# BurnhamG/PyTorch-ScalableFHVAE

Hardware: AMD Instinct MI355X
Metric: segments/sec + ELBO (nats/frame), (B,20,80) fbank (higher is better)
Workload: dtype bf16; 1 GPU; c3: fhvae.FHVAE 2x256 LSTM enc/dec, z1=z2=32, 28k-seq mu2 table, batch 2048; per-GPU batch 2048, T=20, F=80, full train step (fwd+loss+bwd+Adam), intended objective, mu_idx uniform; global_batch=2048, parallelism=single

## Files before the change

pytorch-scalablefhvae_amd/csrc/lstm_bwd_rs.hip:

```cpp
#include <cstdlib>

#include "lstm_cluster_dev.h"
#include "trace.h"

namespace fh {

namespace {

constexpr int kH = 256, kG = 4 * kH, kHU = 64, kNU = 4;
constexpr int kKS = 8;

template <int RT>
__device__ __forceinline__ int rs_xoff(int par, int cluster, int src, int j, int wave, int rt) {
  return ((((((par * 64 + cluster) * kNU + src) * 3 + (j - 1)) * 4 + wave) * RT + rt) << 9);
}

template <int RT>
struct RsCfg {
  static constexpr int SMEM = RT * 16 * 512;
};

template <int RT, bool UM>
__global__ __launch_bounds__(kThreads) void lstm_bwd_layer_rs_kernel(ClBwd p) {
  constexpr int H = kH, G = kG;
  extern __shared__ __attribute__((aligned(16))) char smem[];
  char* Img = smem;
  const int tid = threadIdx.x, lane = tid & 63, wave = tid >> 6;
  const int r = lane & 15, q = lane >> 4;

  const int joined = cluster_join(p.sync, (int*)Img);
  if (joined < 0) return;
  const int info = joined & 255;
  const unsigned ep0 = (unsigned)(joined >> 8) * kSeqEpochs;
  const int cluster = (info >> 5) * (32 / kNU) + (info & 31) / kNU, me = (info & 31) % kNU;
  const int r0 = p.row0 + cluster * p.Mc;
  const int rend = min(p.row0 + p.nrows, r0 + p.Mc);
  if (r0 >= rend) return;
  unsigned* flags = p.sync + kSyncFlags + cluster * 32;
  const int u0 = me * kHU;
  const int uq = u0 + wave * 16 + q * 4;
  const int B = p.B, T = p.T;

  int row[RT];
  int64_t rowc[RT];
#pragma unroll
  for (int rt = 0; rt < RT; ++rt) {
    row[rt] = r0 + rt * 16 + r;
    rowc[rt] = row[rt] < rend ? row[rt] : rend - 1;
  }
  f32x4 dcreg[RT], ccur[RT], dgs[RT][4], own[RT];
#pragma unroll
  for (int rt = 0; rt < RT; ++rt) {
    dcreg[rt] = ccur[rt] = own[rt] = f32x4{0.f, 0.f, 0.f, 0.f};
#pragma unroll
    for (int g = 0; g < 4; ++g) dgs[rt][g] = f32x4{0.f, 0.f, 0.f, 0.f};
  }
  const __amdgpu_buffer_rsrc_t x_rs = make_rsrc(p.xch);
  const float* ext_src = p.d_hs_top;
  int ibase[4], wbase[2];
#pragma unroll
  for (int k3 = 0; k3 < 4; ++k3) {
    ibase[k3] = r * 512 + (((k3 * 4 + q) ^ r) << 4);
  }
#pragma unroll
  for (int g1 = 0; g1 < 2; ++g1)
    wbase[g1] = r * 512 + (((g1 * 8 + 2 * wave + (q >> 1)) ^ r) << 4) + (q & 1) * 8;
  unsigned long long* tl = (p.tlog && cluster == 0 && me == 0) ? p.tlog + (p.tlog_slot ? 256 : 0) : nullptr;
  CL_TLOG(6);

  uint2 gkn[RT][4];
  f32x4 cprevn[RT], extn[RT], ccurn[RT];
  typedef unsigned u32x4v __attribute__((ext_vector_type(4)));
  const bool nt = p.nt != 0;
  auto ld16 = [&](const void* q) -> uint4 {
    if (nt) {
      const u32x4v v = __builtin_nontemporal_load((const u32x4v*)q);
      return uint4{v.x, v.y, v.z, v.w};
    }
    return *(const uint4*)q;
  };
  auto ldf4 = [&](const float* q) -> f32x4 { return nt ? __builtin_nontemporal_load((const f32x4*)q) : *(const f32x4*)q; };
  auto load_epi = [&](int sn) {
    const int t = T - 1 - sn;
#pragma unroll
    for (int rt = 0; rt < RT; ++rt) {
      if constexpr (UM) {
        const u16* gp = p.gates + ((int64_t)t * B + rowc[rt]) * G + uq * 4;
        const uint4 a = ld16(gp), b = ld16(gp + 8);
        gkn[rt][0] = uint2{a.x, a.y}, gkn[rt][1] = uint2{a.z, a.w}, gkn[rt][2] = uint2{b.x, b.y}, gkn[rt][3] = uint2{b.z, b.w};
      } else {
        cl_load_gates(p.gates + ((int64_t)t * B + rowc[rt]) * G, uq, gkn[rt]);
      }
      if (sn == 0) ccurn[rt] = *(const f32x4*)(p.cs + ((int64_t)t * B + rowc[rt]) * H + uq);
      cprevn[rt] = t > 0 ? ldf4(p.cs + ((int64_t)(t - 1) * B + rowc[rt]) * H + uq) : f32x4{0.f, 0.f, 0.f, 0.f};
      f32x4 e = f32x4{0.f, 0.f, 0.f, 0.f};
      if (ext_src) e = ldf4(ext_src + ((int64_t)t * B + rowc[rt]) * H + uq);
      if (sn == 0 && p.d_hn) e += *(const f32x4*)(p.d_hn + rowc[rt] * p.hn_ld + uq);
      extn[rt] = e;
    }
  };
  __syncthreads();
  bf16x8 wreg[kKS][kNU];
#pragma unroll
  for (int ks = 0; ks < kKS; ++ks)
#pragma unroll
    for (int j = 0; j < kNU; ++j) {
      const int unit = ((me + j) & 3) * kHU + wave * 16 + r;
      const int col = (ks >> 1) * H + u0 + (ks & 1) * 32 + q * 8;
      wreg[ks][j] = __builtin_bit_cast(bf16x8, *(const uint4*)(p.w_hh_t[0] + (int64_t)unit * G + col));
    }
  load_epi(0);
  CL_TLOG(7);
  for (int s = 0; s < T; ++s) {
    CL_TLOG(s * 8 + 0);
    const int t = T - 1 - s;
    f32x4 dh[RT];
    CL_TLOG(s * 8 + 1);
    uint2 pin[RT][3];
    if (s > 0) {
      if (!cluster_wait(p.sync, flags, kNU, ep0 + (unsigned)s)) return;
      CL_TLOG(s * 8 + 2);
#pragma unroll
      for (int jj = 1; jj < kNU; ++jj)
#pragma unroll
        for (int rt = 0; rt < RT; ++rt) {
          const u32x2 v = __builtin_amdgcn_raw_buffer_load_b64(x_rs, rs_xoff<RT>((s - 1) & 1, cluster, (me - jj) & 3, jj, wave, rt) + lane * 8, 0, kSc1);
          pin[rt][jj - 1] = uint2{v.x, v.y};
        }
    }
    uint2 gk[RT][4];
    f32x4 cprev[RT];
#pragma unroll
    for (int rt = 0; rt < RT; ++rt) {
#pragma unroll
      for (int g = 0; g < 4; ++g) gk[rt][g] = gkn[rt][g];
      cprev[rt] = cprevn[rt];
      dh[rt] = extn[rt] + own[rt];
      if (s == 0) ccur[rt] = ccurn[rt];
    }
    if (s > 0) {
#pragma unroll
      for (int rt = 0; rt < RT; ++rt)
#pragma unroll
        for (int j = 0; j < 3; ++j) dh[rt] += unpack4(pin[rt][j]);
    }
    __builtin_amdgcn_sched_barrier(0);
    if (s + 1 < T) load_epi(s + 1);
    uint2 dpk[RT][4];
#pragma unroll
    for (int rt = 0; rt < RT; ++rt) {
      f32x4 ig, fg, gg, og;
      if constexpr (UM) {
#pragma unroll
        for (int i = 0; i < 4; ++i) {
          ig[i] = bf2f((u16)(gk[rt][i].x & 0xffff)), fg[i] = bf2f((u16)(gk[rt][i].x >> 16));
          gg[i] = bf2f((u16)(gk[rt][i].y & 0xffff)), og[i] = bf2f((u16)(gk[rt][i].y >> 16));
        }
      } else {
        ig = unpack4(gk[rt][0]), fg = unpack4(gk[rt][1]), gg = unpack4(gk[rt][2]), og = unpack4(gk[rt][3]);
      }
      f32x4 dp[4];
#pragma unroll
      for (int i = 0; i < 4; ++i) {
        const float tc = tanhf_(ccur[rt][i]);
        float dc = dh[rt][i] * og[i] * (1.f - tc * tc);
        if (s > 0) dc += dcreg[rt][i];
        const float d_o = dh[rt][i] * tc;
        const float d_i = dc * gg[i], d_f = dc * cprev[rt][i], d_g = dc * ig[i];
        dcreg[rt][i] = dc * fg[i];
        dp[0][i] = d_i * ig[i] * (1.f - ig[i]);
        dp[1][i] = d_f * fg[i] * (1.f - fg[i]);
        dp[2][i] = d_g * (1.f - gg[i] * gg[i]);
        dp[3][i] = d_o * og[i] * (1.f - og[i]);
      }
      ccur[rt] = cprev[rt];
      const bool live = row[rt] < rend;
#pragma unroll
      for (int g = 0; g < 4; ++g) {
        if (live) dgs[rt][g] += dp[g];
        dpk[rt][g] = pack4(dp[g]);
        *(uint2*)(Img + wbase[g & 1] + (g >> 1) * 256 + rt * 8192) = dpk[rt][g];
      }
    }
    asm volatile("s_waitcnt lgkmcnt(0)\n\ts_barrier" ::: "memory");
    CL_TLOG(s * 8 + 3);
    if (s + 1 < T) {
      f32x4 acc[RT][kNU];
#pragma unroll
      for (int rt = 0; rt < RT; ++rt)
#pragma unroll
        for (int j = 0; j < kNU; ++j) acc[rt][j] = f32x4{0.f, 0.f, 0.f, 0.f};
      bf16x8 bfrag[2][RT];
      auto ifrag = [&](int ks, int buf) {
#pragma unroll
        for (int rt = 0; rt < RT; ++rt)
          bfrag[buf][rt] = __builtin_bit_cast(bf16x8, *(const uint4*)(Img + ibase[ks & 3] + (ks >> 2) * 256 + rt * 8192));
      };
      ifrag(0, 0);
      __builtin_amdgcn_sched_group_barrier(0x100, RT, 0);
#pragma unroll
      for (int ks = 0; ks < kKS; ++ks) {
        if (ks + 1 < kKS) ifrag(ks + 1, (ks + 1) & 1);
#pragma unroll
        for (int j = 0; j < kNU; ++j)
#pragma unroll
          for (int rt = 0; rt < RT; ++rt) acc[rt][j] = __builtin_amdgcn_mfma_f32_16x16x32_bf16(wreg[ks][j], bfrag[ks & 1][rt], acc[rt][j], 0, 0, 0);
        if (ks + 1 < kKS) {
          __builtin_amdgcn_sched_group_barrier(0x008, 1, 0);
          __builtin_amdgcn_sched_group_barrier(0x100, RT, 0);
          __builtin_amdgcn_sched_group_barrier(0x008, RT * kNU - 1, 0);
        } else {
          __builtin_amdgcn_sched_group_barrier(0x008, RT * kNU, 0);
        }
      }
#pragma unroll
      for (int rt = 0; rt < RT; ++rt) {
        own[rt] = acc[rt][0];
#pragma unroll
        for (int j = 1; j < kNU; ++j)
          *(uint2*)((char*)p.xch + rs_xoff<RT>(s & 1, cluster, me, j, wave, rt) + lane * 8) = pack4(acc[rt][j]);
      }
    }
    auto img_chunk = [&](int i) -> uint4 {
      const int c = (wave * RT * 2 + i) * 64 + lane;
      return *(const uint4*)(Img + kc_off<32>(c >> 5, c & 31));
    };
    const uint4 v0 = img_chunk(0), v1 = img_chunk(1), v2 = RT > 1 ? img_chunk(2) : uint4{0u, 0u, 0u, 0u},
                v3 = RT > 1 ? img_chunk(3) : uint4{0u, 0u, 0u, 0u};
    CL_TLOG(s * 8 + 4);
    if (s + 1 < T) cluster_publish(flags, me, ep0 + (unsigned)(s + 1));
    else __syncthreads();
    CL_TLOG(s * 8 + 5);
    auto dg_store = [&](int i, const uint4& v) {
      const int c = (wave * RT * 2 + i) * 64 + lane;
      const int rw = r0 + (c >> 5), cc = c & 31;
      if (rw < rend) {
        u16* dst = p.dg + ((int64_t)t * B + rw) * G + (cc >> 3) * H + u0 + (cc & 7) * 8;
        if (nt)
          __builtin_nontemporal_store(u32x4v{v.x, v.y, v.z, v.w}, (u32x4v*)dst);
        else
          *(uint4*)dst = v;
      }
    };
    dg_store(0, v0);
    dg_store(1, v1);
    if constexpr (RT > 1) {
      dg_store(2, v2);
      dg_store(3, v3);
    }
  }
  if (p.d_xc_zero && me == 0 && wave == 0) {
#pragma unroll
    for (int rt = 0; rt < RT; ++rt)
      if (row[rt] < rend)
        for (int c = q; c < p.Ic; c += 4) p.d_xc_zero[(int64_t)row[rt] * p.Ic + c] = 0.f;
  }
#pragma unroll
  for (int g = 0; g < 4; ++g) {
    f32x4 vs = f32x4{0.f, 0.f, 0.f, 0.f};
#pragma unroll
    for (int rt = 0; rt < RT; ++rt) {
      vs += dgs[rt][g];
      if (p.dgsum && row[rt] < rend) *(f32x4*)(p.dgsum + (int64_t)row[rt] * G + g * H + uq) = dgs[rt][g];
    }
    if (p.db_ih[0] || p.db_hh[0]) db_reduce_add(vs, p.db_ih[0], p.db_hh[0], g * H + uq, lane);
  }
  CL_TLOG((T - 1) * 8 + 7);
}

template <int RT>
int launch_rs(const ClBwd& p, hipStream_t st) {
  if (p.gates_um)
    hipLaunchKernelGGL((lstm_bwd_layer_rs_kernel<RT, true>), dim3(kGrid), dim3(kThreads), RsCfg<RT>::SMEM, st, p);
  else
    hipLaunchKernelGGL((lstm_bwd_layer_rs_kernel<RT, false>), dim3(kGrid), dim3(kThreads), RsCfg<RT>::SMEM, st, p);
  return fh_launch_status();
}

}

int cluster_bwd_layer_rs(const ClBwd& p, hipStream_t st) {
  if (p.NU != kNU || p.Mc > 32 || p.Mc % 16 != 0) return FHVAE_ERR_SHAPE;
  return p.Mc <= 16 ? launch_rs<1>(p, st) : launch_rs<2>(p, st);
}

}
```

Baseline: 1.264 million segments/s.

## Restructure LSTM backward step to precompute gate factors off the critical path

Reorganizes the LSTM backward recurrence so the gate-dependent factors (tanh, sigmoid derivatives, cprev products) are computed for the next step right after its loads are issued, leaving only a few FMAs that depend on the incoming dh. The first timestep is peeled via a compile-time flag, the accumulator zeroing is folded into the first MFMA, and the live-row masking moves out of the loop to the final reduction. The c and ext loads now go through buffer resource descriptors with a zero-range trick for t=0 and a null ext, and the non-temporal load/store path is hardcoded in place of the runtime flag. This raises register pressure from the precomputed factor arrays and removes the option of normal cached accesses.

After: 1.253 million segments/s (median of 2 runs). No clear change (-0.9%).

```diff
diff --git a/pytorch-scalablefhvae_amd/csrc/lstm_bwd_rs.hip b/pytorch-scalablefhvae_amd/csrc/lstm_bwd_rs.hip
--- a/pytorch-scalablefhvae_amd/csrc/lstm_bwd_rs.hip
+++ b/pytorch-scalablefhvae_amd/csrc/lstm_bwd_rs.hip
@@ -1,4 +1,5 @@
 #include <cstdlib>
+#include <type_traits>
 
 #include "lstm_cluster_dev.h"
 #include "trace.h"
@@ -48,10 +49,10 @@
     row[rt] = r0 + rt * 16 + r;
     rowc[rt] = row[rt] < rend ? row[rt] : rend - 1;
   }
-  f32x4 dcreg[RT], ccur[RT], dgs[RT][4], own[RT];
+  f32x4 dcreg[RT], dgs[RT][4], own[RT];
 #pragma unroll
   for (int rt = 0; rt < RT; ++rt) {
-    dcreg[rt] = ccur[rt] = own[rt] = f32x4{0.f, 0.f, 0.f, 0.f};
+    dcreg[rt] = own[rt] = f32x4{0.f, 0.f, 0.f, 0.f};
 #pragma unroll
     for (int g = 0; g < 4; ++g) dgs[rt][g] = f32x4{0.f, 0.f, 0.f, 0.f};
   }
@@ -69,19 +70,21 @@
   CL_TLOG(6);
 
   uint2 gkn[RT][4];
-  f32x4 cprevn[RT], extn[RT], ccurn[RT];
+  f32x4 cprevn[RT], extn[RT], ccur[RT];
   typedef unsigned u32x4v __attribute__((ext_vector_type(4)));
-  const bool nt = p.nt != 0;
   auto ld16 = [&](const void* q) -> uint4 {
-    if (nt) {
-      const u32x4v v = __builtin_nontemporal_load((const u32x4v*)q);
-      return uint4{v.x, v.y, v.z, v.w};
-    }
-    return *(const uint4*)q;
+    const u32x4v v = __builtin_nontemporal_load((const u32x4v*)q);
+    return uint4{v.x, v.y, v.z, v.w};
   };
-  auto ldf4 = [&](const float* q) -> f32x4 { return nt ? __builtin_nontemporal_load((const f32x4*)q) : *(const f32x4*)q; };
+  int coff[RT];
+#pragma unroll
+  for (int rt = 0; rt < RT; ++rt) coff[rt] = (int)((rowc[rt] * H + uq) * 4);
   auto load_epi = [&](int sn) {
     const int t = T - 1 - sn;
+    const __amdgpu_buffer_rsrc_t cs_rs = __builtin_amdgcn_make_buffer_rsrc(const_cast<float*>(p.cs + (int64_t)(t > 0 ? t - 1 : 0) * B * H), 0,
+                                                                            t > 0 ? B * H * 4 : 0, 0x00020000);
+    const __amdgpu_buffer_rsrc_t ext_rs = __builtin_amdgcn_make_buffer_rsrc(const_cast<float*>(ext_src ? ext_src + (int64_t)t * B * H : p.cs), 0,
+                                                                             ext_src ? B * H * 4 : 0, 0x00020000);
 #pragma unroll
     for (int rt = 0; rt < RT; ++rt) {
       if constexpr (UM) {
@@ -91,62 +94,12 @@
       } else {
         cl_load_gates(p.gates + ((int64_t)t * B + rowc[rt]) * G, uq, gkn[rt]);
       }
-      if (sn == 0) ccurn[rt] = *(const f32x4*)(p.cs + ((int64_t)t * B + rowc[rt]) * H + uq);
-      cprevn[rt] = t > 0 ? ldf4(p.cs + ((int64_t)(t - 1) * B + rowc[rt]) * H + uq) : f32x4{0.f, 0.f, 0.f, 0.f};
-      f32x4 e = f32x4{0.f, 0.f, 0.f, 0.f};
-      if (ext_src) e = ldf4(ext_src + ((int64_t)t * B + rowc[rt]) * H + uq);
-      if (sn == 0 && p.d_hn) e += *(const f32x4*)(p.d_hn + rowc[rt] * p.hn_ld + uq);
-      extn[rt] = e;
+      cprevn[rt] = __builtin_bit_cast(f32x4, __builtin_amdgcn_raw_buffer_load_b128(cs_rs, coff[rt], 0, 2));
+      extn[rt] = __builtin_bit_cast(f32x4, __builtin_amdgcn_raw_buffer_load_b128(ext_rs, coff[rt], 0, 2));
     }
   };
-  __syncthreads();
-  bf16x8 wreg[kKS][kNU];
-#pragma unroll
-  for (int ks = 0; ks < kKS; ++ks)
-#pragma unroll
-    for (int j = 0; j < kNU; ++j) {
-      const int unit = ((me + j) & 3) * kHU + wave * 16 + r;
-      const int col = (ks >> 1) * H + u0 + (ks & 1) * 32 + q * 8;
-      wreg[ks][j] = __builtin_bit_cast(bf16x8, *(const uint4*)(p.w_hh_t[0] + (int64_t)unit * G + col));
-    }
-  load_epi(0);
-  CL_TLOG(7);
-  for (int s = 0; s < T; ++s) {
-    CL_TLOG(s * 8 + 0);
-    const int t = T - 1 - s;
-    f32x4 dh[RT];
-    CL_TLOG(s * 8 + 1);
-    uint2 pin[RT][3];
-    if (s > 0) {
-      if (!cluster_wait(p.sync, flags, kNU, ep0 + (unsigned)s)) return;
-      CL_TLOG(s * 8 + 2);
-#pragma unroll
-      for (int jj = 1; jj < kNU; ++jj)
-#pragma unroll
-        for (int rt = 0; rt < RT; ++rt) {
-          const u32x2 v = __builtin_amdgcn_raw_buffer_load_b64(x_rs, rs_xoff<RT>((s - 1) & 1, cluster, (me - jj) & 3, jj, wave, rt) + lane * 8, 0, kSc1);
-          pin[rt][jj - 1] = uint2{v.x, v.y};
-        }
-    }
-    uint2 gk[RT][4];
-    f32x4 cprev[RT];
-#pragma unroll
-    for (int rt = 0; rt < RT; ++rt) {
-#pragma unroll
-      for (int g = 0; g < 4; ++g) gk[rt][g] = gkn[rt][g];
-      cprev[rt] = cprevn[rt];
-      dh[rt] = extn[rt] + own[rt];
-      if (s == 0) ccur[rt] = ccurn[rt];
-    }
-    if (s > 0) {
-#pragma unroll
-      for (int rt = 0; rt < RT; ++rt)
-#pragma unroll
-        for (int j = 0; j < 3; ++j) dh[rt] += unpack4(pin[rt][j]);
-    }
-    __builtin_amdgcn_sched_barrier(0);
-    if (s + 1 < T) load_epi(s + 1);
-    uint2 dpk[RT][4];
+  f32x4 pA[RT], pPo[RT], pPi[RT], pPf[RT], pPg[RT], pF[RT], base[RT];
+  auto prep = [&](const uint2 (&gk)[RT][4], const f32x4 (&cprev)[RT], const f32x4 (&ext)[RT]) {
 #pragma unroll
     for (int rt = 0; rt < RT; ++rt) {
       f32x4 ig, fg, gg, og;
@@ -159,37 +112,95 @@
       } else {
         ig = unpack4(gk[rt][0]), fg = unpack4(gk[rt][1]), gg = unpack4(gk[rt][2]), og = unpack4(gk[rt][3]);
       }
-      f32x4 dp[4];
 #pragma unroll
       for (int i = 0; i < 4; ++i) {
         const float tc = tanhf_(ccur[rt][i]);
-        float dc = dh[rt][i] * og[i] * (1.f - tc * tc);
-        if (s > 0) dc += dcreg[rt][i];
-        const float d_o = dh[rt][i] * tc;
-        const float d_i = dc * gg[i], d_f = dc * cprev[rt][i], d_g = dc * ig[i];
-        dcreg[rt][i] = dc * fg[i];
-        dp[0][i] = d_i * ig[i] * (1.f - ig[i]);
-        dp[1][i] = d_f * fg[i] * (1.f - fg[i]);
-        dp[2][i] = d_g * (1.f - gg[i] * gg[i]);
-        dp[3][i] = d_o * og[i] * (1.f - og[i]);
-      }
+        pA[rt][i] = og[i] * __builtin_fmaf(-tc, tc, 1.f);
+        pPo[rt][i] = tc * __builtin_fmaf(-og[i], og[i], og[i]);
+        pPi[rt][i] = gg[i] * __builtin_fmaf(-ig[i], ig[i], ig[i]);
+        pPf[rt][i] = cprev[rt][i] * __builtin_fmaf(-fg[i], fg[i], fg[i]);
+        pPg[rt][i] = ig[i] * __builtin_fmaf(-gg[i], gg[i], 1.f);
+      }
+      pF[rt] = fg;
       ccur[rt] = cprev[rt];
-      const bool live = row[rt] < rend;
+      base[rt] = ext[rt] + own[rt];
+    }
+  };
+  load_epi(0);
+#pragma unroll
+  for (int rt = 0; rt < RT; ++rt) {
+    ccur[rt] = *(const f32x4*)(p.cs + ((int64_t)(T - 1) * B + rowc[rt]) * H + uq);
+    if (p.d_hn) extn[rt] += *(const f32x4*)(p.d_hn + rowc[rt] * p.hn_ld + uq);
+  }
+  __syncthreads();
+  bf16x8 wreg[kKS][kNU];
+#pragma unroll
+  for (int ks = 0; ks < kKS; ++ks)
+#pragma unroll
+    for (int j = 0; j < kNU; ++j) {
+      const int unit = ((me + j) & 3) * kHU + wave * 16 + r;
+      const int col = (ks >> 1) * H + u0 + (ks & 1) * 32 + q * 8;
+      wreg[ks][j] = __builtin_bit_cast(bf16x8, *(const uint4*)(p.w_hh_t[0] + (int64_t)unit * G + col));
+    }
+  CL_TLOG(7);
+  auto step = [&](auto first_c, const int s) -> bool {
+    constexpr bool FIRST = decltype(first_c)::value;
+    CL_TLOG(s * 8 + 0);
+    const int t = T - 1 - s;
+    f32x4 dh[RT];
+    CL_TLOG(s * 8 + 1);
+    uint2 pin[RT][3];
+    if constexpr (!FIRST) {
+      if (!cluster_wait(p.sync, flags, kNU, ep0 + (unsigned)s)) return false;
+      CL_TLOG(s * 8 + 2);
+#pragma unroll
+      for (int jj = 1; jj < kNU; ++jj)
+#pragma unroll
+        for (int rt = 0; rt < RT; ++rt) {
+          const u32x2 v = __builtin_amdgcn_raw_buffer_load_b64(x_rs, rs_xoff<RT>((s - 1) & 1, cluster, (me - jj) & 3, jj, wave, rt) + lane * 8, 0, kSc1);
+          pin[rt][jj - 1] = uint2{v.x, v.y};
+        }
+    }
+    __builtin_amdgcn_sched_barrier(0);
+    {
+      uint2 gk0[RT][4];
+      f32x4 cp0[RT], ex0[RT];
+#pragma unroll
+      for (int rt = 0; rt < RT; ++rt) {
+#pragma unroll
+        for (int g = 0; g < 4; ++g) gk0[rt][g] = gkn[rt][g];
+        cp0[rt] = cprevn[rt], ex0[rt] = extn[rt];
+      }
+      load_epi(s + 1 < T ? s + 1 : s);
+      prep(gk0, cp0, ex0);
+    }
+    f32x4 dp[RT][4];
+#pragma unroll
+    for (int rt = 0; rt < RT; ++rt) {
+      dh[rt] = base[rt];
+      if constexpr (!FIRST) {
+#pragma unroll
+        for (int j = 0; j < 3; ++j) dh[rt] += unpack4(pin[rt][j]);
+      }
+#pragma unroll
+      for (int i = 0; i < 4; ++i) {
+        const float dc = FIRST ? dh[rt][i] * pA[rt][i] : __builtin_fmaf(dh[rt][i], pA[rt][i], dcreg[rt][i]);
+        dp[rt][0][i] = dc * pPi[rt][i];
+        dp[rt][1][i] = dc * pPf[rt][i];
+        dp[rt][2][i] = dc * pPg[rt][i];
+        dp[rt][3][i] = dh[rt][i] * pPo[rt][i];
+        dcreg[rt][i] = dc * pF[rt][i];
+      }
 #pragma unroll
       for (int g = 0; g < 4; ++g) {
-        if (live) dgs[rt][g] += dp[g];
-        dpk[rt][g] = pack4(dp[g]);
-        *(uint2*)(Img + wbase[g & 1] + (g >> 1) * 256 + rt * 8192) = dpk[rt][g];
+        *(uint2*)(Img + wbase[g & 1] + (g >> 1) * 256 + rt * 8192) = pack4(dp[rt][g]);
+        dgs[rt][g] += dp[rt][g];
       }
     }
     asm volatile("s_waitcnt lgkmcnt(0)\n\ts_barrier" ::: "memory");
     CL_TLOG(s * 8 + 3);
     if (s + 1 < T) {
       f32x4 acc[RT][kNU];
-#pragma unroll
-      for (int rt = 0; rt < RT; ++rt)
-#pragma unroll
-        for (int j = 0; j < kNU; ++j) acc[rt][j] = f32x4{0.f, 0.f, 0.f, 0.f};
       bf16x8 bfrag[2][RT];
       auto ifrag = [&](int ks, int buf) {
 #pragma unroll
@@ -204,7 +215,8 @@
 #pragma unroll
         for (int j = 0; j < kNU; ++j)
 #pragma unroll
-          for (int rt = 0; rt < RT; ++rt) acc[rt][j] = __builtin_amdgcn_mfma_f32_16x16x32_bf16(wreg[ks][j], bfrag[ks & 1][rt], acc[rt][j], 0, 0, 0);
+          for (int rt = 0; rt < RT; ++rt)
+            acc[rt][j] = __builtin_amdgcn_mfma_f32_16x16x32_bf16(wreg[ks][j], bfrag[ks & 1][rt], ks ? acc[rt][j] : f32x4{0.f, 0.f, 0.f, 0.f}, 0, 0, 0);
         if (ks + 1 < kKS) {
           __builtin_amdgcn_sched_group_barrier(0x008, 1, 0);
           __builtin_amdgcn_sched_group_barrier(0x100, RT, 0);
@@ -236,10 +248,7 @@
       const int rw = r0 + (c >> 5), cc = c & 31;
       if (rw < rend) {
         u16* dst = p.dg + ((int64_t)t * B + rw) * G + (cc >> 3) * H + u0 + (cc & 7) * 8;
-        if (nt)
-          __builtin_nontemporal_store(u32x4v{v.x, v.y, v.z, v.w}, (u32x4v*)dst);
-        else
-          *(uint4*)dst = v;
+        __builtin_nontemporal_store(u32x4v{v.x, v.y, v.z, v.w}, (u32x4v*)dst);
       }
     };
     dg_store(0, v0);
@@ -248,7 +257,11 @@
       dg_store(2, v2);
       dg_store(3, v3);
     }
-  }
+    return true;
+  };
+  if (!step(std::true_type{}, 0)) return;
+  for (int s = 1; s < T; ++s)
+    if (!step(std::false_type{}, s)) return;
   if (p.d_xc_zero && me == 0 && wave == 0) {
 #pragma unroll
     for (int rt = 0; rt < RT; ++rt)
@@ -260,8 +273,9 @@
     f32x4 vs = f32x4{0.f, 0.f, 0.f, 0.f};
 #pragma unroll
     for (int rt = 0; rt < RT; ++rt) {
-      vs += dgs[rt][g];
-      if (p.dgsum && row[rt] < rend) *(f32x4*)(p.dgsum + (int64_t)row[rt] * G + g * H + uq) = dgs[rt][g];
+      const bool live = row[rt] < rend;
+      vs += live ? dgs[rt][g] : f32x4{0.f, 0.f, 0.f, 0.f};
+      if (p.dgsum && live) *(f32x4*)(p.dgsum + (int64_t)row[rt] * G + g * H + uq) = dgs[rt][g];
     }
     if (p.db_ih[0] || p.db_hh[0]) db_reduce_add(vs, p.db_ih[0], p.db_hh[0], g * H + uq, lane);
   }
```
